# kallaballa/Poppy

Measured on AMD Instinct MI355X. Metric: morph frames/sec at 1080p, 60-frame sequence; Mpix/s warped, higher is better.
Workload: dtype u8+f32

## Files before the change

poppy_amd/csrc/foreground.cpp:

```cpp
#include "foreground.h"
#include "kernels_prefilter.h"
#include "kernels.h"
#include <algorithm>
#include <cmath>
#include <cstdlib>
#include <cstring>
#include <vector>

namespace poppy_hip {

#define FG_CHK(call)                                                                   \
    do {                                                                               \
        hipError_t e_ = (call);                                                        \
        if (e_ != hipSuccess) { err = std::string(#call) + ": " + hipGetErrorString(e_); return -2; } \
    } while (0)

ForegroundFilter::~ForegroundFilter() {
    release();
    release2();
    if (logtab) (void)hipFree(logtab);
    if (h_easy) (void)hipHostFree(h_easy);
    if (easy_ev) (void)hipEventDestroy(easy_ev);
    if (detail_ev) (void)hipEventDestroy(detail_ev);
}
// ... 20 lines not shown
        FG_CHK(hipMemcpy(logtab, tab.data(), 512 * sizeof(float), hipMemcpyHostToDevice));
        prepared = true;
    }
    if (w == W && h == H) return 0;
    float* keep = logtab;
    release();
    logtab = keep;
    const size_t P = (size_t)w * h;
    FG_CHK(hipMalloc((void**)&d_bgr, P * 3)); FG_CHK(hipMalloc((void**)&grey, P));
    FG_CHK(hipMalloc((void**)&meds, P * 12));
    FG_CHK(hipMalloc((void**)&acc[0], P)); FG_CHK(hipMalloc((void**)&acc[1], P));
    FG_CHK(hipMalloc((void**)&flows, P * kMog2Steps));
    FG_CHK(hipMalloc((void**)&masked, P)); FG_CHK(hipMalloc((void**)&out, P)); FG_CHK(hipMalloc((void**)&lut, 256));
    FG_CHK(hipMalloc((void**)&tmp16, P * 2));
    FG_CHK(hipMalloc((void**)&padded, 2 * median_padded_bytes(w, h)));
    FG_CHK(hipMalloc((void**)&hist, 256 * sizeof(unsigned)));
    FG_CHK(hipMalloc((void**)&med_pres, (2 * median_presence_words(w, h) + 4) * sizeof(uint32_t)));
    if (!h_easy) FG_CHK(hipHostMalloc((void**)&h_easy, 16));
    W = w; H = h;
    return 0;
}

const uint8_t* ForegroundFilter::run_device(const uint8_t* bgr, size_t stride, int w, int h, hipStream_t s, const ForegroundDebugOut* dbg) {
    if (ensure(w, h)) return nullptr;
    const size_t P = (size_t)w * h;
    const int n = (int)P;
    auto chk = [&](hipError_t e, const char* what) { if (e != hipSuccess && err.empty()) err = std::string(what) + ": " + hipGetErrorString(e); };
    auto stage_out = [&](int k, const uint8_t* d) {
        if (dbg && dbg->stages) chk(hipMemcpyAsync(dbg->stages + (size_t)k * P, d, P, hipMemcpyDeviceToHost, s), "stage copy");
    };
    err.clear();
// ... 73 lines not shown
    float* dbg_floats = nullptr;
    if (dbg && dbg->floats) {
        if (!dbgf) chk(hipMalloc((void**)&dbgf, P * 12), "hipMalloc");
        dbg_floats = dbgf;
    }
    if (radial_mask_on && !radial12) {
        std::vector<float> rad;
        radial_mask(w, h, rad);
        chk(hipMalloc((void**)&radial12, P * 4), "hipMalloc");
        if (radial12 && hipMemcpy(radial12, rad.data(), P * 4, hipMemcpyHostToDevice) != hipSuccess) {
            (void)hipFree(radial12); radial12 = nullptr;
            chk(hipErrorUnknown, "radial mask upload");
        }
        if (!radial12) return nullptr;
    }
    launch_fg_tail(grey, acc[cur], logtab, radial_mask_on ? radial12 : nullptr, masked, hist, lut, out, dbg_floats, n, s);
    if (dbg) {
        if (dbg->grey) chk(hipMemcpyAsync(dbg->grey, grey, P, hipMemcpyDeviceToHost, s), "copy");
        if (dbg->masked) chk(hipMemcpyAsync(dbg->masked, masked, P, hipMemcpyDeviceToHost, s), "copy");
        if (dbg->floats && dbgf) chk(hipMemcpyAsync(dbg->floats, dbgf, P * 12, hipMemcpyDeviceToHost, s), "copy");
    }
    chk(hipGetLastError(), "launch");
    return err.empty() ? out : nullptr;
}

int ForegroundFilter::median(const uint8_t* src, int w, int h, int ksize, int form, hipStream_t s, uint8_t* dst) {
    if (!src || !dst || w <= 0 || h <= 0 || ksize < 3 || ksize > 89 || !(ksize & 1) || form < 0 || form > 7) { err = "bad arguments"; return -1; }
    if (ensure(w, h)) return -2;
    const size_t P = (size_t)w * h;
    FG_CHK(hipMemcpyAsync(grey, src, P, hipMemcpyHostToDevice, s));
    launch_pad_cols(grey, padded, w, h, s);
// ... 26 lines not shown
```

poppy_amd/csrc/foreground.h:

```cpp
#pragma once
#include <hip/hip_runtime.h>
#include <cstddef>
#include <cstdint>
#include <string>
#include <vector>

namespace poppy_hip {

struct ForegroundDebugOut {
    uint8_t* grey = nullptr;
    uint8_t* stages = nullptr;
    float* floats = nullptr;
    uint8_t* masked = nullptr;
};

void radial_gradient(int width, int height, std::vector<float>& out);
void gabor_bank(int ks, double sigma, double lambd, double gamma, double psi, std::vector<float>& bank);
void radial_mask(int width, int height, std::vector<float>& out);

class ForegroundFilter {
public:
    ~ForegroundFilter();
    int run(const uint8_t* bgr, size_t stride, int w, int h, hipStream_t s, uint8_t* out, const ForegroundDebugOut* dbg);
    const uint8_t* run_device(const uint8_t* d_bgr, size_t stride, int w, int h, hipStream_t s, const ForegroundDebugOut* dbg);
// ... 25 lines not shown
    void* spec = nullptr;
    unsigned* minmax = nullptr;
    unsigned long long* powsum = nullptr;
    uint8_t *g_tmp = nullptr, *g_out[2] = {nullptr, nullptr};
    void *spec_tmp = nullptr, *spec_out = nullptr;
    int* d_itab[2] = {nullptr, nullptr};
    float* d_wave[2] = {nullptr, nullptr};
    int dft_n[2] = {0, 0}, dft_nf[2] = {0, 0}, dft_factors[2][16] = {};
    int W = 0, H = 0;
    uint8_t *d_bgr = nullptr, *grey = nullptr, *meds = nullptr, *acc[2] = {nullptr, nullptr}, *flows = nullptr;
    uint8_t *masked = nullptr, *out = nullptr, *lut = nullptr;
    uint16_t* tmp16 = nullptr;
    uint8_t* padded = nullptr;
    float *logtab = nullptr, *dbgf = nullptr, *radial12 = nullptr;
    unsigned* hist = nullptr;
    uint32_t* med_pres = nullptr;
    uint32_t* h_easy = nullptr;
    hipEvent_t easy_ev = nullptr;
    hipEvent_t detail_ev = nullptr;
    double detail_px = 0;
    bool prepared = false;
};

}
```

poppy_amd/csrc/foreground2.cpp:

```cpp
#include "foreground.h"
#include "kernels_prefilter.h"
#include "dft_exact.h"
#include <algorithm>
#include <cmath>
#include <cstring>
#include <thread>
#include <vector>

namespace poppy_hip {

#define F2_CHK(call)                                                                   \
    do {                                                                               \
        hipError_t e_ = (call);                                                        \
        if (e_ != hipSuccess) { err = std::string(#call) + ": " + hipGetErrorString(e_); return -2; } \
    } while (0)

static void gaussian_taps(int n, double sigma, std::vector<float>& out) {
    std::vector<double> v(n);
    double sum = 0;
    for (int i = 0; i < n; ++i) { const double x = i - (n - 1) * 0.5; v[i] = std::exp(-(x * x) / (2 * sigma * sigma)); sum += v[i]; }
    out.resize(n);
    for (int i = 0; i < n; ++i) out[i] = (float)(v[i] / sum);
}

// ... 169 lines not shown
    return 0;
}
int ForegroundFilter::detail(const uint8_t* d_gf, int w, int h, hipStream_t s, double* out) {
    const int rc = detail_begin(d_gf, w, h, s);
    return rc ? rc : detail_end(out);
}

const uint8_t* ForegroundFilter::orb_input(const uint8_t* d_gf, int w, int h, int which, hipStream_t s, float* h_us, float* h_gb) {
    if (ensure(w, h) || ensure2(w, h)) return nullptr;
    const int n = w * h;
    launch_unsharp1_gray(d_gf, f_a, f_b, f_c, f_d, taps17, w, h, s);
    if (fft31 && !gabor_direct) launch_gabor_fft31(f_d, fft31, bank31, doubt_list31, f_a, w, h, s);
    else launch_gabor_bank31(f_d, bank31, f_a, w, h, s);
    if (h_us) (void)hipMemcpyAsync(h_us, f_d, (size_t)n * 4, hipMemcpyDeviceToHost, s);
    if (h_gb) (void)hipMemcpyAsync(h_gb, f_a, (size_t)n * 4, hipMemcpyDeviceToHost, s);
    launch_orb_input(f_a, f_d, radial, g_tmp, hist, lut, g_out[which & 1], n, s);
    if (hipGetLastError() != hipSuccess) { err = "orb_input launch failed"; return nullptr; }
    return g_out[which & 1];
}

const float* ForegroundFilter::gabor_field(const uint8_t* d_bgr_packed, int w, int h, hipStream_t s, std::string* err_out) {
    if (err_out) {
        if (w != W || h != H || w != W2 || h != H2) { *err_out = "gabor_field: buffers not prepared for this size"; return nullptr; }
    } else if (ensure(w, h) || ensure2(w, h)) return nullptr;
    launch_u8_to_f32(d_bgr_packed, c3_in, w * h * 3, s);
    if (fft13 && !gabor_direct) launch_gabor_fft13_c3(c3_in, fft13, bank13, doubt_list13, c3_out, w, h, s);
    else launch_gabor_bank13_c3(c3_in, bank13, c3_out, w, h, s);
    if (hipGetLastError() != hipSuccess) { (err_out ? *err_out : err) = "gabor_field launch failed"; return nullptr; }
    return c3_out;
}

// ... 2 lines not shown
```

poppy_amd/csrc/kernels_orb.hip:

```cpp
#include "kernels_orb.h"
#include <cfloat>
#include <climits>

namespace poppy_hip {

__device__ __forceinline__ int reflect101i(int p, int len) {
    if ((unsigned)p < (unsigned)len) return p;
    if (len == 1) return 0;
    do { p = p < 0 ? -p : 2 * len - 2 - p; } while ((unsigned)p >= (unsigned)len);
    return p;
}

__global__ void __launch_bounds__(256) k_orb_level0(const uint8_t* __restrict__ src, int sw, int sh, size_t sstride, uint8_t* __restrict__ atlas, OrbLevel L) {
    int px = blockIdx.x * blockDim.x + threadIdx.x, py = blockIdx.y;
    if (px >= L.w + 2 * kOrbBorder) return;
    int x = reflect101i(px - kOrbBorder, L.w), y = reflect101i(py - kOrbBorder, L.h);
    atlas[L.offset + (size_t)py * L.stride + px] = src[(size_t)y * sstride + x];
}

__device__ __forceinline__ int lin_coeff(int v, double scale, int ssize, int& c0, int& c1, int& kind) {
    double f = scale * ((double)v + 0.5) - 0.5;
    int iv = (int)floor(f);
    if (iv >= 0 && ssize > 1) {
        if (iv < ssize - 1) {
// ... 139 lines not shown
    int sum = 0;
    for (int i = lo; i < hi; ++i) sum += a[i];
    s_part[tid] = sum;
    __syncthreads();
    for (int d = 1; d < 1024; d <<= 1) {
        const int v = tid >= d ? s_part[tid - d] : 0;
        __syncthreads();
        s_part[tid] += v;
        __syncthreads();
    }
    int run = s_part[tid] - sum;
    for (int i = lo; i < hi; ++i) { const int c = a[i]; a[i] = run; run += c; }
    if (tid == 1023) counters[lvl] = s_part[1023];
}

__global__ void __launch_bounds__(256) k_fast_nms_emit(const uint8_t* __restrict__ scores, OrbLevelSet S, NmsLayout lay, const int* __restrict__ rowblk,
                                                       const uint8_t* __restrict__ keepbuf, size_t keep_stride, const int* __restrict__ counters,
                                                       int* __restrict__ cand, int cap) {
    __shared__ int s_cnt[kNmsRows][4];
    const int lvl = blockIdx.z;
    int level_base = 0;
    for (int l = 0; l < lvl; ++l) level_base += min(counters[l], cap);
    const int total_cap = kOrbLevels * cap;
    const OrbLevel L = S.lv[lvl];
    const int W = L.w, nbx = lay.nbx[lvl];
    const int bx = blockIdx.x, y0 = blockIdx.y * kNmsRows;
    if (bx >= nbx || y0 >= L.h) return;
    const int x = bx * 256 + threadIdx.x;
    const unsigned keep = x < W ? keepbuf[(size_t)lvl * keep_stride + (size_t)blockIdx.y * W + x] : 0u;
    if (__syncthreads_or(keep != 0) == 0) return;
    const int lane = threadIdx.x & 63, wv = threadIdx.x >> 6;
    int rank[kNmsRows];
#pragma unroll
    for (int r = 0; r < kNmsRows; ++r) {
        const unsigned long long m = __builtin_amdgcn_ballot_w64((keep >> r) & 1u);
        rank[r] = __builtin_popcountll(m & ((1ull << lane) - 1ull));
        if (lane == 0) s_cnt[r][wv] = __builtin_popcountll(m);
    }
    __syncthreads();
#pragma unroll
    for (int r = 0; r < kNmsRows; ++r)
        if (keep & (1u << r)) {
            int slot = rowblk[lay.base[lvl] + (y0 + r) * nbx + bx] + rank[r];
            for (int w = 0; w < wv; ++w) slot += s_cnt[r][w];
            if (slot < cap && level_base + slot < total_cap) {
                const int pos = (y0 + r) * W + x;
                cand[((size_t)level_base + slot) * 2] = x | ((y0 + r) << 16);
                cand[((size_t)level_base + slot) * 2 + 1] = scores[L.score_offset + pos];
            }
        }
}

__global__ void k_harris(const uint8_t* __restrict__ atlas, OrbLevelSet S, const int* __restrict__ kp, int n, float* __restrict__ resp) {
    int i = blockIdx.x * blockDim.x + threadIdx.x;
    if (i >= n) return;
    const OrbLevel L = S.lv[kp[3 * i]];
    const int st = (int)L.stride;
    const uint8_t* c = atlas + L.offset + (size_t)(kp[3 * i + 2] + kOrbBorder) * L.stride + (kp[3 * i + 1] + kOrbBorder);
    int a = 0, b = 0, cc = 0;
    for (int dy = -3; dy <= 3; ++dy)
        for (int dx = -3; dx <= 3; ++dx) {
            const uint8_t* p = c + dy * st + dx;
            int Ix = ((int)p[1] - p[-1]) * 2 + ((int)p[-st + 1] - p[-st - 1]) + ((int)p[st + 1] - p[st - 1]);
            int Iy = ((int)p[st] - p[-st]) * 2 + ((int)p[st - 1] - p[-st - 1]) + ((int)p[st + 1] - p[-st + 1]);
            a += Ix * Ix; b += Iy * Iy; cc += Ix * Iy;
// ... 208 lines not shown
void launch_fast(const uint8_t* atlas, const OrbLevelSet& S, uint8_t* scores, int threshold, int edge, int* counters, int* cand, int cap, void* scratch, hipStream_t s) {
    const dim3 grid_score((S.lv[0].w + 255) / 256, (S.lv[0].h + kFastRows - 1) / kFastRows, S.n);
    const dim3 grid_nms((S.lv[0].w + 255) / 256, (S.lv[0].h + kNmsRows - 1) / kNmsRows, S.n);
    NmsLayout lay;
    size_t rows = 0, keep = 0;
    for (int l = 0; l < kOrbLevels; ++l) {
        lay.base[l] = (int)rows;
        lay.nbx[l] = l < S.n ? (S.lv[l].w + 255) / 256 : 0;
        if (l < S.n) { rows += (size_t)S.lv[l].h * lay.nbx[l]; keep = std::max(keep, (size_t)((S.lv[l].h + kNmsRows - 1) / kNmsRows) * S.lv[l].w); }
    }
    lay.base[kOrbLevels] = (int)rows;
    for (int l = S.n; l < kOrbLevels; ++l) lay.base[l] = (int)rows;
    const size_t keep_stride = (keep + 255) & ~(size_t)255;
    int* rowblk = (int*)scratch;
    uint8_t* keepbuf = (uint8_t*)scratch + ((rows * sizeof(int) + 255) & ~(size_t)255);
    hipLaunchKernelGGL(k_fast_score, grid_score, dim3(256), 0, s, atlas, S, scores, threshold);
    hipLaunchKernelGGL(k_fast_nms_count, grid_nms, dim3(256), 0, s, scores, S, lay, edge, rowblk, keepbuf, keep_stride);
    hipLaunchKernelGGL(k_fast_nms_scan, dim3(S.n), dim3(1024), 0, s, lay, rowblk, counters);
    hipLaunchKernelGGL(k_fast_nms_emit, grid_nms, dim3(256), 0, s, scores, S, lay, rowblk, keepbuf, keep_stride, counters, cand, cap);
}

void launch_harris(const uint8_t* atlas, const OrbLevelSet& S, const int* kp, int n, float* resp, hipStream_t s) {
    if (n > 0) hipLaunchKernelGGL(k_harris, dim3((n + 63) / 64), dim3(64), 0, s, atlas, S, kp, n, resp);
}
void launch_ic_angle(const uint8_t* atlas, const OrbLevelSet& S, const int* kp, int n, float* angle, hipStream_t s) {
    if (n > 0) hipLaunchKernelGGL(k_ic_angle, dim3(n), dim3(64), 0, s, atlas, S, kp, n, angle);
}

}
```

poppy_amd/csrc/kernels_prefilter.h:

```cpp
#pragma once
#include <hip/hip_runtime.h>
#include <vector>
#include <algorithm>
#include <cstddef>
#include <cstdint>
#include <cstdlib>

inline const char* poppy_experiment_env(const char* name) {
#ifdef POPPY_EXPERIMENTS
    return getenv(name);
#else
    (void)name;
    return nullptr;
#endif
}

namespace poppy_hip {

void launch_bgr2gray(const uint8_t* bgr, size_t stride, uint8_t* gray, int w, int h, hipStream_t s);

constexpr int kMog2Steps = 13;
void launch_mog2_all(const uint8_t* const* imgs, const float* alphaT, const float* prune, int steps, uint8_t* flows, int n_px, hipStream_t s);
void launch_acc_flow(uint8_t* acc, const uint8_t* flow, int n_px, float acc_scale, hipStream_t s, bool first = false);

// ... 5 lines not shown
struct MedianColsGeom { int run, rows, tiles_x, tiles_y; };
MedianColsGeom median_cols_geom(int w, int h);
size_t median_presence_words(int w, int h);
void launch_median_presence(const uint8_t* src_tight, uint32_t* pres, int w, int h, uint32_t* easy_or_null, hipStream_t s);
int median_cols_hint_from_host(const uint8_t* bgr, size_t stride, int w, int h);
void launch_median_cols(const uint8_t* padded_src, uint8_t* dst, uint8_t* padded_next, int w, int h, int ksize, const uint32_t* pres_in, uint32_t* pres_out,
                        int force, hipStream_t s);
int median_cols_min_ksize();
int median_cols_min_ksize_hard();

void launch_gauss23_u8(const uint8_t* src, uint16_t* tmp, uint8_t* dst, int w, int h, hipStream_t s);
void launch_acc_gauss23(const uint8_t* acc, const uint8_t* flow, uint8_t* dst, int w, int h, float acc_scale, hipStream_t s);
bool acc_gauss23_fused_takes(int w, int h);
void launch_acc_gauss23_fused(const uint8_t* acc, const uint8_t* flows, size_t plane, int steps, uint8_t* dst, int w, int h, float acc_scale, hipStream_t s);

void launch_fg_tail(const uint8_t* grey, const uint8_t* fg, const float* d_logtab, const float* radial_or_null, uint8_t* masked, unsigned* hist, uint8_t* lut,
                    uint8_t* out, float* dbg_or_null, int n_px, hipStream_t s);

void launch_strip_blur(const uint8_t* canvas, uint8_t* out, int cw, uint32_t* tmp, const int* d_taps, int n, int rx, int ry, int rw, int rh, hipStream_t s);

void launch_equalize_from_hist(const uint8_t* src, const unsigned* hist, uint8_t* lut, uint8_t* out, int n_px, hipStream_t s);

void launch_unsharp1_gray(const uint8_t* gf, float* f32, float* tmp, float* diff, float* out, const float* d_taps17, int w, int h, hipStream_t s);
void launch_gabor_bank31(const float* src, const double* d_bank, float* dst, int w, int h, hipStream_t s);
void launch_gabor_bank13_c3(const float* src, const double* d_bank, float* dst, int w, int h, hipStream_t s);
std::vector<double> gabor_fft_tables(const std::vector<float>& bank, int ks);
bool gabor_fft_prepare();
bool gabor_fft_doubt(unsigned long long out[3]);
double gabor_band_unit();
void launch_gabor_fft31(const float* src, const double* d_tables, const double* d_bank, unsigned* d_list, float* dst, int w, int h, hipStream_t s);
void launch_gabor_fft13_c3(const float* src, const double* d_tables, const double* d_bank, unsigned* d_list, float* dst, int w, int h, hipStream_t s);
void launch_u8_to_f32(const uint8_t* src, float* dst, int n, hipStream_t s);
void launch_orb_input(const float* gb, const float* us, const float* radial, uint8_t* tmp_u8, unsigned* hist, uint8_t* lut, uint8_t* out,
                      int n_px, hipStream_t s);
struct DftPlanDev { int n, nf; int factors[16]; const int* itab; const float2* wave; };
void launch_dft2d_exact(const float2* src, float2* tmp, float2* dst, int n, int m, const DftPlanDev& rows, const DftPlanDev& cols, hipStream_t s);
void launch_pad_complex(const uint8_t* src, float2* dst, int w, int h, int n, int m, unsigned* minmax, unsigned long long* powsum, hipStream_t s);
void launch_spectrum_log(const float2* spec, float* mag, const float* d_logtab, unsigned* minmax, int n, int m, int nc, int mc, hipStream_t s);
void launch_spectrum_bytes(const float* mag, const unsigned* minmax, int nc, int mc, unsigned long long* powsum, hipStream_t s);

}
```

poppy_amd/csrc/kernels_prefilter.hip:

```cpp
#include "kernels_prefilter.h"
#include <cstdlib>
#include "pyramid_device.h"

namespace poppy_hip {

__global__ void __launch_bounds__(256) k_bgr2gray(const uint8_t* __restrict__ bgr, size_t stride, uint8_t* __restrict__ gray, int W, int H) {
    const int x = blockIdx.x * 256 + threadIdx.x, y = blockIdx.y;
    if (x >= W) return;
    const uint8_t* p = bgr + (size_t)y * stride + (size_t)x * 3;
    gray[(size_t)y * W + x] = (uint8_t)((p[0] * 3735 + p[1] * 19235 + p[2] * 9798 + (1 << 14)) >> 15);
}
void launch_bgr2gray(const uint8_t* bgr, size_t stride, uint8_t* gray, int w, int h, hipStream_t s) {
    hipLaunchKernelGGL(k_bgr2gray, dim3((w + 255) / 256, h), dim3(256), 0, s, bgr, stride, gray, w, h);
}

constexpr int kMog2Modes = 5;

typedef float mog2_vec __attribute__((ext_vector_type(16)));
__device__ __forceinline__ int mog2_step_body(float (&w)[kMog2Modes], float (&v)[kMog2Modes], float (&mu)[kMog2Modes], int& nmodes,
                                              float data, float alphaT, float prune);
__device__ __noinline__ mog2_vec mog2_step(mog2_vec m, float data, float alphaT, float prune) {
    float w[kMog2Modes], v[kMog2Modes], mu[kMog2Modes];
#pragma unroll
    for (int k = 0; k < kMog2Modes; ++k) { w[k] = m[k]; v[k] = m[kMog2Modes + k]; mu[k] = m[2 * kMog2Modes + k]; }
// ... 577 lines not shown
        const int add = t >= d ? s_h[t - d] : 0;
        __syncthreads();
        s_h[t] += add;
        __syncthreads();
    }
    const float scale = __fdiv_rn(256 - 1.f, (float)(total - hf));
    const int sum = s_h[t] - s_h[first];
    lut[t] = t <= first ? (uint8_t)0 : sat_u8(cv_round_x86((float)sum * scale));
}
__global__ void __launch_bounds__(256) k_apply_lut(const uint8_t* __restrict__ src, const uint8_t* __restrict__ lut, uint8_t* __restrict__ dst, int n) {
    __shared__ uint8_t l[256];
    l[threadIdx.x] = lut[threadIdx.x];
    __syncthreads();
    for (int p = blockIdx.x * 256 + threadIdx.x; p < n; p += gridDim.x * 256) dst[p] = l[src[p]];
}
void launch_equalize_from_hist(const uint8_t* src, const unsigned* hist, uint8_t* lut, uint8_t* out, int n_px, hipStream_t s) {
    const int blocks = std::min((n_px + 255) / 256, 2048);
    hipLaunchKernelGGL(k_equalize_lut, dim3(1), dim3(256), 0, s, hist, n_px, lut);
    hipLaunchKernelGGL(k_apply_lut, dim3(blocks), dim3(256), 0, s, src, lut, out, n_px);
}
void launch_fg_tail(const uint8_t* grey, const uint8_t* fg, const float* d_logtab, const float* radial_or_null, uint8_t* masked, unsigned* hist, uint8_t* lut,
                    uint8_t* out, float* dbg_or_null, int n_px, hipStream_t s) {
    (void)hipMemsetAsync(hist, 0, 256 * sizeof(unsigned), s);
    const int blocks = std::min((n_px + 255) / 256, 2048);
    hipLaunchKernelGGL(k_fg_mask, dim3(blocks), dim3(256), 0, s, grey, fg, d_logtab, radial_or_null, masked, hist, dbg_or_null, n_px);
    hipLaunchKernelGGL(k_equalize_lut, dim3(1), dim3(256), 0, s, hist, n_px, lut);
    hipLaunchKernelGGL(k_apply_lut, dim3(blocks), dim3(256), 0, s, masked, lut, out, n_px);
}

}
```

poppy_amd/csrc/kernels_prefilter2.hip:

```cpp
#include "kernels_prefilter.h"
#include <algorithm>
#include "pyramid_device.h"

namespace poppy_hip {

__global__ void __launch_bounds__(256) k_u8_to_f32(const uint8_t* __restrict__ src, float* __restrict__ dst, int n) {
    const int i = blockIdx.x * 256 + threadIdx.x;
    if (i < n) dst[i] = (float)src[i] * kInv255 + 0.f;
}
__global__ void __launch_bounds__(256) k_sep_row(const float* __restrict__ src, float* __restrict__ dst, const float* __restrict__ taps, int ksize, int W, int H) {
    const int x = blockIdx.x * 256 + threadIdx.x, y = blockIdx.y;
    if (x >= W) return;
    const float* row = src + (size_t)y * W;
    const int r = ksize >> 1;
    float acc = row[reflect101(x - r, W)] * taps[0];
    for (int k = 1; k < ksize; ++k) acc = row[reflect101(x - r + k, W)] * taps[k] + acc;
    dst[(size_t)y * W + x] = acc;
}
__global__ void __launch_bounds__(256) k_sep_col_diff(const float* __restrict__ src, const float* __restrict__ tmp, float* __restrict__ diff,
                                                      const float* __restrict__ taps, int ksize, int W, int H) {
    const int x = blockIdx.x * 256 + threadIdx.x, y = blockIdx.y;
    if (x >= W) return;
    const int r = ksize >> 1;
    float acc = taps[r] * tmp[(size_t)y * W + x] + 0.f;
// ... 16 lines not shown
                                                       int W, int H, float amount, float threshold) {
    const int x = blockIdx.x * 256 + threadIdx.x, y = blockIdx.y;
    if (x >= W) return;
    float d;
    if (W == 1 || H == 1) {
        const int len = W + H - 1, i = (H == 1) ? x : y;
        float p0 = diff[i > 0 ? i - 1 : i], p1 = diff[i], p2 = diff[i < len - 1 ? i + 1 : i];
        d = __builtin_amdgcn_fmed3f(p0, p1, p2);
    } else d = med9(diff, W, H, x, y);
    const size_t p = (size_t)y * W + x;
    float v = src[p];
    const double n2 = (double)d * (double)d + (double)d * (double)d + (double)d * (double)d;
    if (sqrt(n2) >= (double)threshold) v = v + amount * d;
    out[p] = v * 0.299f + (v * 0.587f + v * 0.114f);
}
void launch_unsharp1_gray(const uint8_t* gf, float* f32, float* tmp, float* diff, float* out, const float* d_taps17, int w, int h, hipStream_t s) {
    const int n = w * h;
    dim3 grid((w + 255) / 256, h);
    hipLaunchKernelGGL(k_u8_to_f32, dim3((n + 255) / 256), dim3(256), 0, s, gf, f32, n);
    hipLaunchKernelGGL(k_sep_row, grid, dim3(256), 0, s, f32, tmp, d_taps17, 17, w, h);
    hipLaunchKernelGGL(k_sep_col_diff, grid, dim3(256), 0, s, f32, tmp, diff, d_taps17, 17, w, h);
    hipLaunchKernelGGL(k_unsharp1_gray, grid, dim3(256), 0, s, f32, diff, out, w, h, 6.f, 0.1f);
}

template <int K, int CN>
__global__ void __launch_bounds__(256) k_gabor_bank(const float* __restrict__ src, const double* __restrict__ bank, float* __restrict__ dst, int W, int H) {
    constexpr int R = K / 2, TX = 32, TY = 8, SX = TX + 2 * R, SY = TY + 2 * R;
    __shared__ float tile[SY * SX];
    const int tx0 = blockIdx.x * TX, ty0 = blockIdx.y * TY, ch = blockIdx.z;
    for (int i = threadIdx.x; i < SY * SX; i += 256) {
        const int r = i / SX, c = i - r * SX;
// ... 32 lines not shown
__global__ void __launch_bounds__(256) k_orb_input(const float* __restrict__ gb, const float* __restrict__ us, const float* __restrict__ radial,
                                                   uint8_t* __restrict__ out, unsigned* __restrict__ hist, int n) {
    __shared__ unsigned lh[256];
    lh[threadIdx.x] = 0;
    __syncthreads();
    for (int p = blockIdx.x * 256 + threadIdx.x; p < n; p += gridDim.x * 256) {
        float g = gb[p] * us[p];
        g = g * radial[p];
        const uint8_t o = sat_u8(cv_round_x86(g * 255.f + 0.f));
        out[p] = o;
        atomicAdd(&lh[o], 1u);
    }
    __syncthreads();
    if (lh[threadIdx.x]) atomicAdd(&hist[threadIdx.x], lh[threadIdx.x]);
}
void launch_orb_input(const float* gb, const float* us, const float* radial, uint8_t* tmp_u8, unsigned* hist, uint8_t* lut, uint8_t* out,
                      int n_px, hipStream_t s) {
    (void)hipMemsetAsync(hist, 0, 256 * sizeof(unsigned), s);
    const int blocks = std::min((n_px + 255) / 256, 2048);
    hipLaunchKernelGGL(k_orb_input, dim3(blocks), dim3(256), 0, s, gb, us, radial, tmp_u8, hist, n_px);
    launch_equalize_from_hist(tmp_u8, hist, lut, out, n_px, s);
}

__device__ __forceinline__ float cv_log32f_dev(float x, const float* __restrict__ tab) {
    const float A0 = 0.3333333333333333333333333f, A1 = -0.5f, A2 = 1.f;
    const float ln2 = (float)0.69314718055994530941723212145818;
    const int i0 = __float_as_int(x);
    const float bf = __int_as_float((i0 & ((1 << 15) - 1)) | (127 << 23));
    const int idx = (i0 >> 14) & 510;
    const float y0 = (float)(((i0 >> 23) & 0xff) - 127) * ln2 + tab[idx];
    const float x0 = (bf - 1.f) * tab[idx + 1] + (idx == 510 ? -1.f / 512 : 0.f);
    return ((A0 * x0 + A1) * x0 + A2) * x0 + y0;
// ... 310 lines not shown
```

Baseline: 8144.

## Fuse FAST scoring with NMS, tile unsharp filter, vectorize setup histogram tails

Adds a flat-grid fused FAST score plus NMS kernel that stages pyramid pixels and scores in shared memory, replacing two separate passes. Replaces the four-kernel unsharp grayscale chain with a single tiled kernel doing separable blur, diff and 3x3 median in LDS. Vectorizes the fg-mask and orb-input histogram tails with 4-pixel loads and wave-aggregated LDS atomics, and uses double-banked histogram bins to avoid a separate memset. An env var restores the old paths; the tile kernel keeps a near-threshold exact double check for bit parity, at the cost of added complexity.

Result: slower. 8050 (-1.2%).

```diff
diff --git a/poppy_amd/csrc/foreground.cpp b/poppy_amd/csrc/foreground.cpp
--- a/poppy_amd/csrc/foreground.cpp
+++ b/poppy_amd/csrc/foreground.cpp
@@ -58,7 +58,8 @@
     FG_CHK(hipMalloc((void**)&masked, P)); FG_CHK(hipMalloc((void**)&out, P)); FG_CHK(hipMalloc((void**)&lut, 256));
     FG_CHK(hipMalloc((void**)&tmp16, P * 2));
     FG_CHK(hipMalloc((void**)&padded, 2 * median_padded_bytes(w, h)));
-    FG_CHK(hipMalloc((void**)&hist, 256 * sizeof(unsigned)));
+    FG_CHK(hipMalloc((void**)&hist, 512 * sizeof(unsigned)));
+    bins = SetupBins{hist, 0, false};
     FG_CHK(hipMalloc((void**)&med_pres, (2 * median_presence_words(w, h) + 4) * sizeof(uint32_t)));
     if (!h_easy) FG_CHK(hipHostMalloc((void**)&h_easy, 16));
     W = w; H = h;
@@ -162,7 +163,7 @@
         }
         if (!radial12) return nullptr;
     }
-    launch_fg_tail(grey, acc[cur], logtab, radial_mask_on ? radial12 : nullptr, masked, hist, lut, out, dbg_floats, n, s);
+    launch_fg_tail(grey, acc[cur], logtab, radial_mask_on ? radial12 : nullptr, masked, hist, lut, out, dbg_floats, n, s, &bins);
     if (dbg) {
         if (dbg->grey) chk(hipMemcpyAsync(dbg->grey, grey, P, hipMemcpyDeviceToHost, s), "copy");
         if (dbg->masked) chk(hipMemcpyAsync(dbg->masked, masked, P, hipMemcpyDeviceToHost, s), "copy");
diff --git a/poppy_amd/csrc/foreground.h b/poppy_amd/csrc/foreground.h
--- a/poppy_amd/csrc/foreground.h
+++ b/poppy_amd/csrc/foreground.h
@@ -4,6 +4,7 @@
 #include <cstdint>
 #include <string>
 #include <vector>
+#include "kernels_prefilter.h"
 
 namespace poppy_hip {
 
@@ -63,6 +64,7 @@
     uint8_t* padded = nullptr;
     float *logtab = nullptr, *dbgf = nullptr, *radial12 = nullptr;
     unsigned* hist = nullptr;
+    SetupBins bins;
     uint32_t* med_pres = nullptr;
     uint32_t* h_easy = nullptr;
     hipEvent_t easy_ev = nullptr;
diff --git a/poppy_amd/csrc/foreground2.cpp b/poppy_amd/csrc/foreground2.cpp
--- a/poppy_amd/csrc/foreground2.cpp
+++ b/poppy_amd/csrc/foreground2.cpp
@@ -207,7 +207,7 @@
     else launch_gabor_bank31(f_d, bank31, f_a, w, h, s);
     if (h_us) (void)hipMemcpyAsync(h_us, f_d, (size_t)n * 4, hipMemcpyDeviceToHost, s);
     if (h_gb) (void)hipMemcpyAsync(h_gb, f_a, (size_t)n * 4, hipMemcpyDeviceToHost, s);
-    launch_orb_input(f_a, f_d, radial, g_tmp, hist, lut, g_out[which & 1], n, s);
+    launch_orb_input(f_a, f_d, radial, g_tmp, hist, lut, g_out[which & 1], n, s, &bins);
     if (hipGetLastError() != hipSuccess) { err = "orb_input launch failed"; return nullptr; }
     return g_out[which & 1];
 }
diff --git a/poppy_amd/csrc/hist_device.h b/poppy_amd/csrc/hist_device.h
--- /dev/null
+++ b/poppy_amd/csrc/hist_device.h
@@ -0,0 +1,25 @@
+#pragma once
+#include <hip/hip_runtime.h>
+#include <cstdint>
+
+namespace poppy_hip {
+
+constexpr int kHistRounds = 3;
+__device__ __forceinline__ void hist_add_wave(unsigned* lh, unsigned o, bool valid) {
+    const int lane = (int)__builtin_amdgcn_mbcnt_hi(~0u, __builtin_amdgcn_mbcnt_lo(~0u, 0u));
+    bool pending = valid;
+#pragma unroll
+    for (int r = 0; r < kHistRounds; ++r) {
+        const unsigned long long pm = __builtin_amdgcn_ballot_w64(pending);
+        if (pm == 0) break;
+        const int leader = __builtin_ctzll(pm);
+        const unsigned lv = (unsigned)__builtin_amdgcn_readlane((int)o, leader);
+        const bool mine = pending && o == lv;
+        const unsigned long long m = __builtin_amdgcn_ballot_w64(mine);
+        if (lane == leader) atomicAdd(&lh[lv], (unsigned)__builtin_popcountll(m));
+        if (mine) pending = false;
+    }
+    if (pending) atomicAdd(&lh[o], 1u);
+}
+
+}
diff --git a/poppy_amd/csrc/kernels_orb.hip b/poppy_amd/csrc/kernels_orb.hip
--- a/poppy_amd/csrc/kernels_orb.hip
+++ b/poppy_amd/csrc/kernels_orb.hip
@@ -1,4 +1,6 @@
 #include "kernels_orb.h"
+#include "kernels_prefilter.h"
+#include <algorithm>
 #include <cfloat>
 #include <climits>
 
@@ -177,20 +179,18 @@
     if (tid == 1023) counters[lvl] = s_part[1023];
 }
 
-__global__ void __launch_bounds__(256) k_fast_nms_emit(const uint8_t* __restrict__ scores, OrbLevelSet S, NmsLayout lay, const int* __restrict__ rowblk,
-                                                       const uint8_t* __restrict__ keepbuf, size_t keep_stride, const int* __restrict__ counters,
-                                                       int* __restrict__ cand, int cap) {
-    __shared__ int s_cnt[kNmsRows][4];
-    const int lvl = blockIdx.z;
+__device__ __forceinline__ void fast_nms_emit_block(const uint8_t* __restrict__ scores, const OrbLevelSet& S, const NmsLayout& lay, const int* __restrict__ rowblk,
+                                                    const uint8_t* __restrict__ keepbuf, size_t keep_stride, const int* __restrict__ counters,
+                                                    int* __restrict__ cand, int cap, int (*s_cnt)[4], int lvl, int bx, int by) {
     int level_base = 0;
     for (int l = 0; l < lvl; ++l) level_base += min(counters[l], cap);
     const int total_cap = kOrbLevels * cap;
     const OrbLevel L = S.lv[lvl];
     const int W = L.w, nbx = lay.nbx[lvl];
-    const int bx = blockIdx.x, y0 = blockIdx.y * kNmsRows;
+    const int y0 = by * kNmsRows;
     if (bx >= nbx || y0 >= L.h) return;
     const int x = bx * 256 + threadIdx.x;
-    const unsigned keep = x < W ? keepbuf[(size_t)lvl * keep_stride + (size_t)blockIdx.y * W + x] : 0u;
+    const unsigned keep = x < W ? keepbuf[(size_t)lvl * keep_stride + (size_t)by * W + x] : 0u;
     if (__syncthreads_or(keep != 0) == 0) return;
     const int lane = threadIdx.x & 63, wv = threadIdx.x >> 6;
     int rank[kNmsRows];
@@ -212,6 +212,97 @@
                 cand[((size_t)level_base + slot) * 2 + 1] = scores[L.score_offset + pos];
             }
         }
+}
+__global__ void __launch_bounds__(256) k_fast_nms_emit(const uint8_t* __restrict__ scores, OrbLevelSet S, NmsLayout lay, const int* __restrict__ rowblk,
+                                                       const uint8_t* __restrict__ keepbuf, size_t keep_stride, const int* __restrict__ counters,
+                                                       int* __restrict__ cand, int cap) {
+    __shared__ int s_cnt[kNmsRows][4];
+    fast_nms_emit_block(scores, S, lay, rowblk, keepbuf, keep_stride, counters, cand, cap, s_cnt, blockIdx.z, blockIdx.x, blockIdx.y);
+}
+
+struct FastBlocks { int base[kOrbLevels + 1]; };
+__device__ __forceinline__ void fast_block_of(const FastBlocks& fb, const NmsLayout& lay, int b, int& lvl, int& bx, int& by) {
+    lvl = 0;
+#pragma unroll
+    for (int l = 1; l < kOrbLevels; ++l) lvl += b >= fb.base[l] ? 1 : 0;
+    const int local = b - fb.base[lvl], nbx = lay.nbx[lvl];
+    by = local / nbx; bx = local - by * nbx;
+}
+__global__ void __launch_bounds__(256) k_fast_nms_emit_flat(const uint8_t* __restrict__ scores, OrbLevelSet S, NmsLayout lay, FastBlocks fb, const int* __restrict__ rowblk,
+                                                            const uint8_t* __restrict__ keepbuf, size_t keep_stride, const int* __restrict__ counters,
+                                                            int* __restrict__ cand, int cap) {
+    __shared__ int s_cnt[kNmsRows][4];
+    int lvl, bx, by;
+    fast_block_of(fb, lay, blockIdx.x, lvl, bx, by);
+    fast_nms_emit_block(scores, S, lay, rowblk, keepbuf, keep_stride, counters, cand, cap, s_cnt, lvl, bx, by);
+}
+
+constexpr int kFfSrcCols = 256 + 8, kFfSrcRows = kNmsRows + 8;
+constexpr int kFfScCols = 256 + 2, kFfScStride = 260;
+__global__ void __launch_bounds__(256) k_fast_nms_fused(const uint8_t* __restrict__ atlas, OrbLevelSet S, NmsLayout lay, FastBlocks fb, uint8_t* __restrict__ scores,
+                                                        int threshold, int edge, int atlas_dword_ok, int* __restrict__ rowblk, uint8_t* __restrict__ keepbuf, size_t keep_stride) {
+    __shared__ uint32_t s_src[kFfSrcRows * (kFfSrcCols / 4)];
+    __shared__ uint8_t s_sc[(kNmsRows + 2) * kFfScStride];
+    __shared__ int s_cnt[kNmsRows][4];
+    const int tid = threadIdx.x;
+    int lvl, bx, by;
+    fast_block_of(fb, lay, blockIdx.x, lvl, bx, by);
+    const OrbLevel L = S.lv[lvl];
+    const int W = L.w, H = L.h, nbx = lay.nbx[lvl];
+    const int x0 = bx * 256, y0 = by * kNmsRows, x = x0 + tid;
+    const bool dead = W <= 2 * edge || H <= 2 * edge || y0 >= H - edge || y0 + kNmsRows <= edge || x0 >= W - edge;
+    unsigned keep = 0;
+    if (!dead) {
+        const int stride = (int)L.stride, px0 = x0 - 4 + kOrbBorder;
+        const uint8_t* base = atlas + L.offset + (size_t)(y0 - 4 + kOrbBorder) * L.stride + px0;
+        uint8_t* const src_b = reinterpret_cast<uint8_t*>(s_src);
+        if (atlas_dword_ok && (stride & 3) == 0 && (L.offset & 3) == 0) {
+            for (int i = tid; i < kFfSrcRows * (kFfSrcCols / 4); i += 256) {
+                const int r = i / (kFfSrcCols / 4), q = i - r * (kFfSrcCols / 4);
+                s_src[i] = px0 + 4 * q + 4 <= stride ? *reinterpret_cast<const uint32_t*>(base + (size_t)r * L.stride + 4 * q) : 0u;
+            }
+        } else {
+            for (int i = tid; i < kFfSrcRows * kFfSrcCols; i += 256) {
+                const int r = i / kFfSrcCols, c = i - r * kFfSrcCols;
+                src_b[i] = px0 + c < stride ? base[(size_t)r * L.stride + c] : (uint8_t)0;
+            }
+        }
+        __syncthreads();
+        const int xs_lo = max(3, edge - 1), xs_hi = min(W - 3, W - edge + 1), ys_lo = max(3, edge - 1), ys_hi = min(H - 3, H - edge + 1);
+        for (int i = tid; i < (kNmsRows + 2) * kFfScCols; i += 256) {
+            const int sr = i / kFfScCols, scol = i - sr * kFfScCols;
+            const int xs = x0 - 1 + scol, ys = y0 - 1 + sr;
+            int v = 0;
+            if (xs >= xs_lo && xs < xs_hi && ys >= ys_lo && ys < ys_hi) v = fast_score_at(src_b + (sr + 3) * kFfSrcCols + scol + 3, kFfSrcCols, threshold);
+            s_sc[sr * kFfScStride + scol] = (uint8_t)v;
+        }
+        __syncthreads();
+        if (x >= edge && x < W - edge) {
+#pragma unroll
+            for (int r = 0; r < kNmsRows; ++r) {
+                const int y = y0 + r;
+                if (y >= edge && y < H - edge) {
+                    const uint8_t* p = s_sc + (r + 1) * kFfScStride + tid + 1;
+                    constexpr int T = kFfScStride;
+                    const int v = p[0];
+                    if (v != 0 && v > p[-1] && v > p[1] && v > p[-T - 1] && v > p[-T] && v > p[-T + 1] && v > p[T - 1] && v > p[T] && v > p[T + 1]) {
+                        keep |= 1u << r;
+                        scores[L.score_offset + (size_t)y * W + x] = (uint8_t)v;
+                    }
+                }
+            }
+        }
+    }
+    if (x < W) keepbuf[(size_t)lvl * keep_stride + (size_t)by * W + x] = (uint8_t)keep;
+    const int lane = tid & 63, wv = tid >> 6;
+#pragma unroll
+    for (int r = 0; r < kNmsRows; ++r) {
+        const unsigned long long m = __builtin_amdgcn_ballot_w64((keep >> r) & 1u);
+        if (lane == 0) s_cnt[r][wv] = __builtin_popcountll(m);
+    }
+    __syncthreads();
+    if (tid < kNmsRows && y0 + tid < H)
+        rowblk[lay.base[lvl] + (y0 + tid) * nbx + bx] = s_cnt[tid][0] + s_cnt[tid][1] + s_cnt[tid][2] + s_cnt[tid][3];
 }
 
 __global__ void k_harris(const uint8_t* __restrict__ atlas, OrbLevelSet S, const int* __restrict__ kp, int n, float* __restrict__ resp) {
@@ -450,6 +541,20 @@
     const size_t keep_stride = (keep + 255) & ~(size_t)255;
     int* rowblk = (int*)scratch;
     uint8_t* keepbuf = (uint8_t*)scratch + ((rows * sizeof(int) + 255) & ~(size_t)255);
+    if (!setup_plain()) {
+        FastBlocks fb;
+        int blocks = 0;
+        for (int l = 0; l < kOrbLevels; ++l) {
+            fb.base[l] = blocks;
+            if (l < S.n) blocks += lay.nbx[l] * ((S.lv[l].h + kNmsRows - 1) / kNmsRows);
+        }
+        fb.base[kOrbLevels] = blocks;
+        if (blocks <= 0) return;
+        hipLaunchKernelGGL(k_fast_nms_fused, dim3(blocks), dim3(256), 0, s, atlas, S, lay, fb, scores, threshold, edge, (int)(((uintptr_t)atlas & 3) == 0), rowblk, keepbuf, keep_stride);
+        hipLaunchKernelGGL(k_fast_nms_scan, dim3(S.n), dim3(1024), 0, s, lay, rowblk, counters);
+        hipLaunchKernelGGL(k_fast_nms_emit_flat, dim3(blocks), dim3(256), 0, s, scores, S, lay, fb, rowblk, keepbuf, keep_stride, counters, cand, cap);
+        return;
+    }
     hipLaunchKernelGGL(k_fast_score, grid_score, dim3(256), 0, s, atlas, S, scores, threshold);
     hipLaunchKernelGGL(k_fast_nms_count, grid_nms, dim3(256), 0, s, scores, S, lay, edge, rowblk, keepbuf, keep_stride);
     hipLaunchKernelGGL(k_fast_nms_scan, dim3(S.n), dim3(1024), 0, s, lay, rowblk, counters);
diff --git a/poppy_amd/csrc/kernels_prefilter.h b/poppy_amd/csrc/kernels_prefilter.h
--- a/poppy_amd/csrc/kernels_prefilter.h
+++ b/poppy_amd/csrc/kernels_prefilter.h
@@ -43,8 +43,14 @@
 bool acc_gauss23_fused_takes(int w, int h);
 void launch_acc_gauss23_fused(const uint8_t* acc, const uint8_t* flows, size_t plane, int steps, uint8_t* dst, int w, int h, float acc_scale, hipStream_t s);
 
+struct SetupBins { unsigned* d = nullptr; int bank = 0; bool zero = false; };
 void launch_fg_tail(const uint8_t* grey, const uint8_t* fg, const float* d_logtab, const float* radial_or_null, uint8_t* masked, unsigned* hist, uint8_t* lut,
-                    uint8_t* out, float* dbg_or_null, int n_px, hipStream_t s);
+                    uint8_t* out, float* dbg_or_null, int n_px, hipStream_t s, SetupBins* bins);
+bool setup_plain();
+constexpr int kSetupTailThreads = 1024;
+int setup_tail_blocks(int n_px);
+unsigned* setup_tail_begin(SetupBins& b, hipStream_t s);
+void setup_tail_end(SetupBins& b, const uint8_t* src, uint8_t* out, int n_px, hipStream_t s);
 
 void launch_strip_blur(const uint8_t* canvas, uint8_t* out, int cw, uint32_t* tmp, const int* d_taps, int n, int rx, int ry, int rw, int rh, hipStream_t s);
 
@@ -61,7 +67,7 @@
 void launch_gabor_fft13_c3(const float* src, const double* d_tables, const double* d_bank, unsigned* d_list, float* dst, int w, int h, hipStream_t s);
 void launch_u8_to_f32(const uint8_t* src, float* dst, int n, hipStream_t s);
 void launch_orb_input(const float* gb, const float* us, const float* radial, uint8_t* tmp_u8, unsigned* hist, uint8_t* lut, uint8_t* out,
-                      int n_px, hipStream_t s);
+                      int n_px, hipStream_t s, SetupBins* bins);
 struct DftPlanDev { int n, nf; int factors[16]; const int* itab; const float2* wave; };
 void launch_dft2d_exact(const float2* src, float2* tmp, float2* dst, int n, int m, const DftPlanDev& rows, const DftPlanDev& cols, hipStream_t s);
 void launch_pad_complex(const uint8_t* src, float2* dst, int w, int h, int n, int m, unsigned* minmax, unsigned long long* powsum, hipStream_t s);
diff --git a/poppy_amd/csrc/kernels_prefilter.hip b/poppy_amd/csrc/kernels_prefilter.hip
--- a/poppy_amd/csrc/kernels_prefilter.hip
+++ b/poppy_amd/csrc/kernels_prefilter.hip
@@ -1,6 +1,7 @@
 #include "kernels_prefilter.h"
 #include <cstdlib>
 #include "pyramid_device.h"
+#include "hist_device.h"
 
 namespace poppy_hip {
 
@@ -615,13 +616,116 @@
     __syncthreads();
     for (int p = blockIdx.x * 256 + threadIdx.x; p < n; p += gridDim.x * 256) dst[p] = l[src[p]];
 }
+__device__ __forceinline__ uint8_t fg_mask_px(unsigned gb, unsigned fb, bool has_radial, float rad, const float* ltab, float ln20) {
+    const float g = (float)gb * kInv255 + 0.f;
+    float m = (float)fb * kInv255 + 0.f;
+    if (has_radial) m = m * rad;
+    const float lin = m * 19.f + 1.f;
+    const float lg = cv_log32f(lin, ltab);
+    const float fin = __fdiv_rn(lg, ln20);
+    const float mk = g * fin;
+    return sat_u8(cv_round_x86(mk * 255.f + 0.f));
+}
+__global__ void __launch_bounds__(kSetupTailThreads) k_fg_mask4(const uint8_t* __restrict__ grey, const uint8_t* __restrict__ fg, const float* __restrict__ tab,
+                                                  const float* __restrict__ radial, uint8_t* __restrict__ masked, unsigned* __restrict__ hist, int n) {
+    __shared__ unsigned lh[256];
+    __shared__ float ltab[512];
+    if (threadIdx.x < 256) lh[threadIdx.x] = 0;
+    if (threadIdx.x < 512) ltab[threadIdx.x] = tab[threadIdx.x];
+    __syncthreads();
+    const float ln20 = cv_log32f(20.f, ltab);
+    const int groups = (n + 3) >> 2;
+    for (int base = blockIdx.x * kSetupTailThreads; base < groups; base += gridDim.x * kSetupTailThreads) {
+        const int q = base + threadIdx.x, p = 4 * q;
+        const int cnt = q < groups ? min(4, n - p) : 0;
+        unsigned o[4] = {0, 0, 0, 0};
+        if (cnt == 4) {
+            const uint32_t g4 = *reinterpret_cast<const uint32_t*>(grey + p), f4 = *reinterpret_cast<const uint32_t*>(fg + p);
+            float4 r4 = make_float4(0.f, 0.f, 0.f, 0.f);
+            if (radial) r4 = *reinterpret_cast<const float4*>(radial + p);
+            o[0] = fg_mask_px(g4 & 255u, f4 & 255u, radial != nullptr, r4.x, ltab, ln20);
+            o[1] = fg_mask_px((g4 >> 8) & 255u, (f4 >> 8) & 255u, radial != nullptr, r4.y, ltab, ln20);
+            o[2] = fg_mask_px((g4 >> 16) & 255u, (f4 >> 16) & 255u, radial != nullptr, r4.z, ltab, ln20);
+            o[3] = fg_mask_px(g4 >> 24, f4 >> 24, radial != nullptr, r4.w, ltab, ln20);
+            *reinterpret_cast<uint32_t*>(masked + p) = o[0] | o[1] << 8 | o[2] << 16 | o[3] << 24;
+        } else {
+            for (int k = 0; k < cnt; ++k) {
+                o[k] = fg_mask_px(grey[p + k], fg[p + k], radial != nullptr, radial ? radial[p + k] : 0.f, ltab, ln20);
+                masked[p + k] = (uint8_t)o[k];
+            }
+        }
+#pragma unroll
+        for (int k = 0; k < 4; ++k) hist_add_wave(lh, o[k], k < cnt);
+    }
+    __syncthreads();
+    if (threadIdx.x < 256 && lh[threadIdx.x]) atomicAdd(&hist[threadIdx.x], lh[threadIdx.x]);
+}
+
+__global__ void __launch_bounds__(256) k_equalize_apply(const uint8_t* __restrict__ src, const unsigned* __restrict__ hist, unsigned* __restrict__ other_bank,
+                                                        int total, uint8_t* __restrict__ dst, int n) {
+    __shared__ int s_h[256];
+    __shared__ int s_wsum[4], s_wfirst[4];
+    __shared__ uint8_t l[256];
+    const int t = threadIdx.x, lane = t & 63, w = t >> 6;
+    if (blockIdx.x == 0) other_bank[t] = 0;
+    const int h = (int)hist[t];
+    s_h[t] = h;
+    int incl = h;
+#pragma unroll
+    for (int d = 1; d < 64; d <<= 1) {
+        const int v = __shfl_up(incl, d);
+        if (lane >= d) incl += v;
+    }
+    const unsigned long long nz = __builtin_amdgcn_ballot_w64(h != 0);
+    if (lane == 63) s_wsum[w] = incl;
+    if (lane == 0) s_wfirst[w] = nz ? w * 64 + __builtin_ctzll(nz) : 255;
+    __syncthreads();
+    const int first = min(min(s_wfirst[0], s_wfirst[1]), min(s_wfirst[2], s_wfirst[3]));
+    int pre = incl;
+    for (int k = 0; k < w; ++k) pre += s_wsum[k];
+    const int hf = s_h[first];
+    if (hf == total) l[t] = (uint8_t)first;
+    else {
+        const float scale = __fdiv_rn(256 - 1.f, (float)(total - hf));
+        const int sum = pre - hf;
+        l[t] = t <= first ? (uint8_t)0 : sat_u8(cv_round_x86((float)sum * scale));
+    }
+    __syncthreads();
+    const int groups = n >> 2;
+    for (int q = blockIdx.x * 256 + t; q < groups; q += gridDim.x * 256) {
+        const uint32_t v = *reinterpret_cast<const uint32_t*>(src + 4 * (size_t)q);
+        *reinterpret_cast<uint32_t*>(dst + 4 * (size_t)q) = (uint32_t)l[v & 255u] | (uint32_t)l[(v >> 8) & 255u] << 8 | (uint32_t)l[(v >> 16) & 255u] << 16 | (uint32_t)l[v >> 24] << 24;
+    }
+    if (blockIdx.x == 0 && t < (n & 3)) dst[4 * groups + t] = l[src[4 * groups + t]];
+}
+int setup_tail_blocks(int n_px) { return std::max(1, std::min((((n_px + 3) >> 2) + kSetupTailThreads - 1) / kSetupTailThreads, 256)); }
+unsigned* setup_tail_begin(SetupBins& b, hipStream_t s) {
+    if (!b.zero && hipMemsetAsync(b.d, 0, 512 * sizeof(unsigned), s) != hipSuccess) return nullptr;
+    b.zero = false;
+    return b.d + 256 * b.bank;
+}
+void setup_tail_end(SetupBins& b, const uint8_t* src, uint8_t* out, int n_px, hipStream_t s) {
+    const int blocks = std::max(1, std::min((((n_px + 3) >> 2) + 255) / 256, 512));
+    hipLaunchKernelGGL(k_equalize_apply, dim3(blocks), dim3(256), 0, s, src, b.d + 256 * b.bank, b.d + 256 * (b.bank ^ 1), n_px, out, n_px);
+    if (hipPeekAtLastError() == hipSuccess) { b.zero = true; b.bank ^= 1; }
+}
+
 void launch_equalize_from_hist(const uint8_t* src, const unsigned* hist, uint8_t* lut, uint8_t* out, int n_px, hipStream_t s) {
     const int blocks = std::min((n_px + 255) / 256, 2048);
     hipLaunchKernelGGL(k_equalize_lut, dim3(1), dim3(256), 0, s, hist, n_px, lut);
     hipLaunchKernelGGL(k_apply_lut, dim3(blocks), dim3(256), 0, s, src, lut, out, n_px);
 }
 void launch_fg_tail(const uint8_t* grey, const uint8_t* fg, const float* d_logtab, const float* radial_or_null, uint8_t* masked, unsigned* hist, uint8_t* lut,
-                    uint8_t* out, float* dbg_or_null, int n_px, hipStream_t s) {
+                    uint8_t* out, float* dbg_or_null, int n_px, hipStream_t s, SetupBins* bins) {
+    const bool aligned = (((uintptr_t)grey | (uintptr_t)fg | (uintptr_t)masked | (uintptr_t)out) & 3) == 0 && ((uintptr_t)radial_or_null & 15) == 0;
+    if (!dbg_or_null && aligned && bins && !setup_plain()) {
+        unsigned* bank = setup_tail_begin(*bins, s);
+        if (!bank) return;
+        hipLaunchKernelGGL(k_fg_mask4, dim3(setup_tail_blocks(n_px)), dim3(kSetupTailThreads), 0, s, grey, fg, d_logtab, radial_or_null, masked, bank, n_px);
+        setup_tail_end(*bins, masked, out, n_px, s);
+        return;
+    }
+    if (bins) bins->zero = false;
     (void)hipMemsetAsync(hist, 0, 256 * sizeof(unsigned), s);
     const int blocks = std::min((n_px + 255) / 256, 2048);
     hipLaunchKernelGGL(k_fg_mask, dim3(blocks), dim3(256), 0, s, grey, fg, d_logtab, radial_or_null, masked, hist, dbg_or_null, n_px);
diff --git a/poppy_amd/csrc/kernels_prefilter2.hip b/poppy_amd/csrc/kernels_prefilter2.hip
--- a/poppy_amd/csrc/kernels_prefilter2.hip
+++ b/poppy_amd/csrc/kernels_prefilter2.hip
@@ -1,6 +1,7 @@
 #include "kernels_prefilter.h"
 #include <algorithm>
 #include "pyramid_device.h"
+#include "hist_device.h"
 
 namespace poppy_hip {
 
@@ -54,7 +55,111 @@
     if (sqrt(n2) >= (double)threshold) v = v + amount * d;
     out[p] = v * 0.299f + (v * 0.587f + v * 0.114f);
 }
+constexpr int kG1Tx = 64, kG1Ty = 32;
+constexpr int kG1Sr = kG1Ty + 18, kG1Ss = kG1Tx + 24, kG1Rs = kG1Tx + 4, kG1Dr = kG1Ty + 2;
+typedef float g1f4 __attribute__((ext_vector_type(4)));
+
+__global__ void __launch_bounds__(256) k_unsharp1_gray_tile(const uint8_t* __restrict__ gf, float* __restrict__ out, const float* __restrict__ taps,
+                                                            int W, int H, int tiles_x, int dword_ok, float amount, float threshold) {
+    __shared__ __attribute__((aligned(16))) float S[kG1Sr * kG1Ss];
+    __shared__ __attribute__((aligned(16))) float R[kG1Sr * kG1Rs];
+    __shared__ __attribute__((aligned(16))) float D[kG1Dr * kG1Rs];
+    const int tid = threadIdx.x;
+    const int tile_y = blockIdx.x / tiles_x, tile_x = blockIdx.x - tile_y * tiles_x;
+    const int tx0 = tile_x * kG1Tx, ty0 = tile_y * kG1Ty;
+    float g[17];
+#pragma unroll
+    for (int k = 0; k < 17; ++k) g[k] = taps[k];
+    if (dword_ok && tx0 >= 12 && tx0 + kG1Tx + 12 <= W && ty0 >= 9 && ty0 + kG1Ty + 9 <= H) {
+        const uint8_t* base = gf + (size_t)(ty0 - 9) * W + (tx0 - 12);
+        for (int i = tid; i < kG1Sr * (kG1Ss / 4); i += 256) {
+            const int r = i / (kG1Ss / 4), q = i - r * (kG1Ss / 4);
+            const uint32_t b = *reinterpret_cast<const uint32_t*>(base + (size_t)r * W + 4 * q);
+            g1f4 v;
+            v.x = (float)(b & 255u) * kInv255 + 0.f; v.y = (float)((b >> 8) & 255u) * kInv255 + 0.f;
+            v.z = (float)((b >> 16) & 255u) * kInv255 + 0.f; v.w = (float)(b >> 24) * kInv255 + 0.f;
+            *(g1f4*)(S + r * kG1Ss + 4 * q) = v;
+        }
+    } else {
+        for (int i = tid; i < kG1Sr * (kG1Tx + 18); i += 256) {
+            const int r = i / (kG1Tx + 18), c = i - r * (kG1Tx + 18);
+            const int yy = reflect101(ty0 - 9 + r, H), xx = reflect101(tx0 - 9 + c, W);
+            S[r * kG1Ss + 3 + c] = (float)gf[(size_t)yy * W + xx] * kInv255 + 0.f;
+        }
+    }
+    __syncthreads();
+    for (int i = tid; i < kG1Sr * (kG1Rs / 4); i += 256) {
+        const int r = i / (kG1Rs / 4), j0 = 4 * (i - r * (kG1Rs / 4));
+        const float* sp = S + r * kG1Ss + j0 + 3;
+        float v[20];
+#pragma unroll
+        for (int k = 0; k < 20; ++k) v[k] = k + j0 + 3 < kG1Ss ? sp[k] : 0.f;
+        g1f4 acc;
+        float* a = (float*)&acc;
+#pragma unroll
+        for (int o = 0; o < 4; ++o) {
+            a[o] = v[o] * g[0];
+#pragma unroll
+            for (int k = 1; k < 17; ++k) a[o] = v[o + k] * g[k] + a[o];
+        }
+        *(g1f4*)(R + r * kG1Rs + j0) = acc;
+    }
+    __syncthreads();
+    for (int i = tid; i < (kG1Dr / 2) * (kG1Rs / 4); i += 256) {
+        const int qi = i / (kG1Rs / 4), j0 = 4 * (i - qi * (kG1Rs / 4)), q0 = 2 * qi;
+        g1f4 rr[18];
+#pragma unroll
+        for (int k = 0; k < 18; ++k) rr[k] = *(const g1f4*)(R + (q0 + k) * kG1Rs + j0);
+#pragma unroll
+        for (int jr = 0; jr < 2; ++jr) {
+            g1f4 acc = g[8] * rr[8 + jr] + 0.f;
+#pragma unroll
+            for (int k = 1; k <= 8; ++k) acc = g[8 + k] * (rr[8 + jr + k] + rr[8 + jr - k]) + acc;
+            const float* sc = S + (q0 + jr + 8) * kG1Ss + j0 + 11;
+            g1f4 d;
+            d.x = sc[0] - acc.x; d.y = sc[1] - acc.y; d.z = sc[2] - acc.z; d.w = j0 + 14 < kG1Ss ? sc[3] - acc.w : 0.f;
+            *(g1f4*)(D + (q0 + jr) * kG1Rs + j0) = d;
+        }
+    }
+    __syncthreads();
+    const float t2f = threshold * threshold;
+    for (int it = 0; it < kG1Ty / 4; ++it) {
+        const int lx = tid & 63, ly = (tid >> 6) + 4 * it;
+        const int x = tx0 + lx, y = ty0 + ly;
+        if (x >= W || y >= H) continue;
+        const int jm = (x > 0 ? lx : lx + 1), jc = lx + 1, jp = (x < W - 1 ? lx + 2 : lx + 1);
+        const float* r0 = D + (y > 0 ? ly : ly + 1) * kG1Rs;
+        const float* r1 = D + (ly + 1) * kG1Rs;
+        const float* r2 = D + (y < H - 1 ? ly + 2 : ly + 1) * kG1Rs;
+        const float a0 = r0[jm], a1 = r0[jc], a2 = r0[jp], b0 = r1[jm], b1 = r1[jc], b2 = r1[jp], c0 = r2[jm], c1 = r2[jc], c2 = r2[jp];
+        const float lo = fmaxf(fmaxf(fminf(fminf(a0, b0), c0), fminf(fminf(a1, b1), c1)), fminf(fminf(a2, b2), c2));
+        const float mi = __builtin_amdgcn_fmed3f(__builtin_amdgcn_fmed3f(a0, b0, c0), __builtin_amdgcn_fmed3f(a1, b1, c1), __builtin_amdgcn_fmed3f(a2, b2, c2));
+        const float hi = fminf(fminf(fmaxf(fmaxf(a0, b0), c0), fmaxf(fmaxf(a1, b1), c1)), fmaxf(fmaxf(a2, b2), c2));
+        const float d = __builtin_amdgcn_fmed3f(lo, mi, hi);
+        float v = S[(ly + 9) * kG1Ss + lx + 12];
+        const float f = d * d + d * d + d * d;
+        bool sharpen = f > t2f;
+        if (__builtin_amdgcn_ballot_w64(fabsf(f - t2f) <= t2f * 1e-5f) != 0) {
+            const double n2 = (double)d * (double)d + (double)d * (double)d + (double)d * (double)d;
+            sharpen = sqrt(n2) >= (double)threshold;
+        }
+        if (sharpen) v = v + amount * d;
+        out[(size_t)y * W + x] = v * 0.299f + (v * 0.587f + v * 0.114f);
+    }
+}
+
+bool setup_plain() {
+    const char* e = getenv("POPPY_SETUP_PLAIN");
+    return e && *e && *e != '0';
+}
+
 void launch_unsharp1_gray(const uint8_t* gf, float* f32, float* tmp, float* diff, float* out, const float* d_taps17, int w, int h, hipStream_t s) {
+    if (w > 1 && h > 1 && !setup_plain()) {
+        const int tiles_x = (w + kG1Tx - 1) / kG1Tx, tiles_y = (h + kG1Ty - 1) / kG1Ty;
+        const int dword_ok = (w & 3) == 0 && ((uintptr_t)gf & 3) == 0;
+        hipLaunchKernelGGL(k_unsharp1_gray_tile, dim3(tiles_x * tiles_y), dim3(256), 0, s, gf, out, d_taps17, w, h, tiles_x, dword_ok, 6.f, 0.1f);
+        return;
+    }
     const int n = w * h;
     dim3 grid((w + 255) / 256, h);
     hipLaunchKernelGGL(k_u8_to_f32, dim3((n + 255) / 256), dim3(256), 0, s, gf, f32, n);
@@ -117,8 +222,45 @@
     __syncthreads();
     if (lh[threadIdx.x]) atomicAdd(&hist[threadIdx.x], lh[threadIdx.x]);
 }
+__device__ __forceinline__ unsigned orb_input_px(float gb, float us, float radial) {
+    float g = gb * us;
+    g = g * radial;
+    return sat_u8(cv_round_x86(g * 255.f + 0.f));
+}
+__global__ void __launch_bounds__(kSetupTailThreads) k_orb_input4(const float* __restrict__ gb, const float* __restrict__ us, const float* __restrict__ radial,
+                                                    uint8_t* __restrict__ out, unsigned* __restrict__ hist, int n) {
+    __shared__ unsigned lh[256];
+    if (threadIdx.x < 256) lh[threadIdx.x] = 0;
+    __syncthreads();
+    const int groups = (n + 3) >> 2;
+    for (int base = blockIdx.x * kSetupTailThreads; base < groups; base += gridDim.x * kSetupTailThreads) {
+        const int q = base + threadIdx.x, p = 4 * q;
+        const int cnt = q < groups ? min(4, n - p) : 0;
+        unsigned o[4] = {0, 0, 0, 0};
+        if (cnt == 4) {
+            const float4 a = *reinterpret_cast<const float4*>(gb + p), b = *reinterpret_cast<const float4*>(us + p), c = *reinterpret_cast<const float4*>(radial + p);
+            o[0] = orb_input_px(a.x, b.x, c.x); o[1] = orb_input_px(a.y, b.y, c.y); o[2] = orb_input_px(a.z, b.z, c.z); o[3] = orb_input_px(a.w, b.w, c.w);
+            *reinterpret_cast<uint32_t*>(out + p) = o[0] | o[1] << 8 | o[2] << 16 | o[3] << 24;
+        } else {
+            for (int k = 0; k < cnt; ++k) { o[k] = orb_input_px(gb[p + k], us[p + k], radial[p + k]); out[p + k] = (uint8_t)o[k]; }
+        }
+#pragma unroll
+        for (int k = 0; k < 4; ++k) hist_add_wave(lh, o[k], k < cnt);
+    }
+    __syncthreads();
+    if (threadIdx.x < 256 && lh[threadIdx.x]) atomicAdd(&hist[threadIdx.x], lh[threadIdx.x]);
+}
 void launch_orb_input(const float* gb, const float* us, const float* radial, uint8_t* tmp_u8, unsigned* hist, uint8_t* lut, uint8_t* out,
-                      int n_px, hipStream_t s) {
+                      int n_px, hipStream_t s, SetupBins* bins) {
+    const bool aligned = (((uintptr_t)gb | (uintptr_t)us | (uintptr_t)radial) & 15) == 0 && (((uintptr_t)tmp_u8 | (uintptr_t)out) & 3) == 0;
+    if (aligned && bins && !setup_plain()) {
+        unsigned* bank = setup_tail_begin(*bins, s);
+        if (!bank) return;
+        hipLaunchKernelGGL(k_orb_input4, dim3(setup_tail_blocks(n_px)), dim3(kSetupTailThreads), 0, s, gb, us, radial, tmp_u8, bank, n_px);
+        setup_tail_end(*bins, tmp_u8, out, n_px, s);
+        return;
+    }
+    if (bins) bins->zero = false;
     (void)hipMemsetAsync(hist, 0, 256 * sizeof(unsigned), s);
     const int blocks = std::min((n_px + 255) / 256, 2048);
     hipLaunchKernelGGL(k_orb_input, dim3(blocks), dim3(256), 0, s, gb, us, radial, tmp_u8, hist, n_px);
```
